# fakerlove1/HPFG

Measured on AMD Instinct MI355X. Metric: labeled+unlabeled images/sec/node, U-Net 224x224 ACDC-shaped (Mean-Teacher step), higher is better.
Workload: dtype bf16x3 (fp32 storage; products as split-bf16 MFMA hi*hi+hi*lo+lo*hi, fp32 accumulate); 1 GPU; mean_teacher_unet_224x224 (BASELINE configs[1]): U-Net 1ch->4cls, 8 labelled + 8 unlabelled per GPU, student fwd+bwd + train-mode teacher fwd + CE/Dice/MSE + SGD + EMA; size=224, hipgraph=True, sync_bn=False, parallelism=dp1, math=bf16x3

## Files before the change

### hpfg_amd/_lib.py

```python
from __future__ import annotations

import ctypes as C
import os
import threading

_HERE = os.path.dirname(os.path.abspath(__file__))
LIB_PATH = os.path.join(_HERE, "lib", "libhpfg_hip.so")

BN_MEAN, BN_RSTD, BN_SCALE, BN_SHIFT, BN_K1, BN_K2, BN_K3, BN_SPARE, BN_ROWS = range(9)
ACT_NONE, ACT_PLAIN, ACT_STRIDED, ACT_BNACT, ACT_BNACT_POOL, ACT_UP2X, ACT_DZ, ACT_SPLIT16, ACT_UPBWD = range(9)
OPT_CONV_THIN, OPT_FIRST_MFMA, OPT_FIRST_WGRAD, OPT_NARROW_DEEP = 0, 1, 2, 3
LOSS_NSUM = 32
ACC_MAX_SHARDS = 8
VERSION = 132
MATH_F32, MATH_BF16X3 = 0, 1


class HipLibraryError(RuntimeError):
    pass


class Act(C.Structure):
    _fields_ = [("z", C.c_void_p), ("bn", C.c_void_p), ("aux", C.c_void_p), ("mode", C.c_int32), ("C", C.c_int32),
                ("Hs", C.c_int32), ("Ws", C.c_int32), ("pstride", C.c_int32), ("aux_pstride", C.c_int32),
                ("bn_stride", C.c_int32), ("bn_coff", C.c_int32), ("sn", C.c_int32), ("sc", C.c_int32), ("sy", C.c_int32),
                ("sx", C.c_int32), ("drop_p", C.c_float), ("drop_seed", C.c_uint32), ("drop_mask", C.c_void_p), ("seed_dev", C.c_void_p),
                ("bn_acc", C.c_void_p), ("bn_gamma", C.c_void_p), ("bn_beta", C.c_void_p), ("bn_count", C.c_float), ("bn_eps", C.c_float),
                ("bn_shards", C.c_int32), ("reserved1", C.c_int32)]


class ConvArgs(C.Structure):
    _fields_ = [("a0", Act), ("a1", Act), ("wpk", C.c_void_p), ("bias", C.c_void_p), ("out", C.c_void_p),
                ("stat_partials", C.c_void_p), ("out_pstride", C.c_int32), ("Cout", C.c_int32), ("CoutPad", C.c_int32),
                ("N", C.c_int32), ("H", C.c_int32), ("W", C.c_int32), ("taps", C.c_int32), ("math", C.c_int32),
                ("bwd_stats", C.c_int32), ("bwd_of", Act), ("out2", C.c_void_p), ("out_split", C.c_int32), ("out2_pstride", C.c_int32),
                ("stat_acc", C.c_void_p), ("stat_shards", C.c_int32), ("reserved2", C.c_int32), ("stage_out", C.c_void_p), ("side_sums", C.c_void_p)]


class WgradArgs(C.Structure):
    _fields_ = [("a0", Act), ("a1", Act), ("g", Act), ("slab", C.c_void_p), ("dw_oihw", C.c_void_p), ("Cin", C.c_int32),
                ("CinPad", C.c_int32), ("Cout", C.c_int32), ("CoutPad", C.c_int32), ("N", C.c_int32), ("H", C.c_int32),
                ("W", C.c_int32), ("taps", C.c_int32), ("S", C.c_int32), ("math", C.c_int32), ("defer_reduce", C.c_int32)]


# ... 165 lines not shown
    "hpfg_neck_pool_fwd": (_i, [_p, _i, _i, _i, _i, _i, _i, _p, _p, _p]),
    "hpfg_neck_pool_bwd": (_i, [_p, _p, _i, _i, _i, _i, _i, _p, _p]),
    "hpfg_l2norm_fwd": (_i, [_p, _i, _i, _i, _i, _i, _p, _p, _p]),
    "hpfg_l2norm_bwd": (_i, [_p, _p, _p, _i, _i, _i, _i, _i, _p, _p, _p]),
    "hpfg_ntxent_rows": (_i, [_p, _i, _f, _p, _p, _p]),
}

_lock = threading.Lock()
_lib = None


def load() -> C.CDLL:
    global _lib
    if _lib is not None:
        return _lib
    with _lock:
        if _lib is not None:
            return _lib
        if not os.path.exists(LIB_PATH):
            raise HipLibraryError(
                f"{LIB_PATH} not found: build it with `python -c 'import __graft_entry__ as g; g.build()'` "
                f"or `make -C hpfg_amd/csrc`. There is no CPU fallback for the HIP path.")
        lib = C.CDLL(LIB_PATH)
        for name, (res, args) in PROTOTYPES.items():
            fn = getattr(lib, name)
            fn.restype = res
            fn.argtypes = args
        if lib.hpfg_version() != VERSION:
            raise HipLibraryError(f"libhpfg_hip.so version {lib.hpfg_version()} != binding version {VERSION}; rebuild")
        if os.environ.get("HPFG_FIRST_WGRAD", "1") == "0":
            lib.hpfg_set_option(OPT_FIRST_WGRAD, 0)
        if os.environ.get("HPFG_NARROW_DEEP") is not None:
            lib.hpfg_set_option(OPT_NARROW_DEEP, int(os.environ["HPFG_NARROW_DEEP"]))
        _lib = lib
    return _lib


def check(rc: int, what: str):
    if rc != 0:
        msg = load().hpfg_last_error().decode("utf-8", "replace")
        raise HipLibraryError(f"{what} failed (rc={rc}): {msg}")


def ptr(t):
    return None if t is None else t.data_ptr()


def none_act() -> Act:
    return Act()
```

### hpfg_amd/csrc/conv_bf16_kernel.h

```cpp
#pragma once
#include <stdlib.h>
#include "stage.h"

namespace hpfg_conv16 {

using namespace hpfg_stage;

template <int TH_, int TW_, int WM_, int WN_, int NI_, int TAPS_, int KC_>
struct Cfg {
  static constexpr int TH = TH_, TW = TW_, WM = WM_, WN = WN_, NI = NI_, TAPS = TAPS_, KC = KC_;
  static constexpr int MI = TH * TW / 16 / WM;
  static constexpr int BN = 16 * NI * WN;
  static constexpr int HALO = TAPS == 9 ? 1 : 0;
  static constexpr int HP = TH + 2 * HALO, WP = TW + 2 * HALO;
  static constexpr int RS = TW == 16 ? WP : (TAPS == 9 ? 24 : 8);
  static constexpr int NSLOT = (HP * RS + 15) / 16 * 16;
  static constexpr int NG = KC / 8;
  static constexpr int PLANE = NSLOT * 16;
  static constexpr int BUF_BYTES = NG * 2 * PLANE;
  static constexpr int KSTEPS = TAPS == 1 ? 1 : (KC == 32 ? 9 : 5);
  static constexpr int NPIECE = HP * WP * NG;
  static constexpr int NLD = (NPIECE + 255) / 256;
  static_assert(WM * WN == 4, "4 waves per workgroup");
  static_assert(256 % NG == 0, "a thread must keep one channel group");
  static_assert(KC == 32 || (KC == 16 && TAPS == 9), "two-tap K packing only for 3x3");
  static_assert(TAPS == 1 || NLD + 2 <= KSTEPS, "stage pipeline must fit into the k-steps of a chunk");
};

__device__ __forceinline__ int clampi(int v, int lo, int hi) { return min(max(v, lo), hi); }

struct Piece {
  int ly, lx, lds, ok;
};
template <class C>
__device__ __forceinline__ Piece make_piece(int tid, int i) {
  Piece q;
  const int idx = tid + i * 256;
  const int pix = idx / C::NG, g = idx % C::NG;
  q.ok = idx < C::NPIECE;
  q.ly = pix / C::WP - C::HALO;
  q.lx = pix % C::WP - C::HALO;
  q.lds = (g * 2) * C::PLANE + ((pix / C::WP) * C::RS + pix % C::WP) * 16;
  return q;
}

template <class C, int KIND = HPFG_KIND_PLAIN, bool SIDE_ON = false>
__device__ __forceinline__ void store_piece(unsigned char* buf, const Piece& q, const f32x4& v0, const f32x4& v1, const HpfgConvArgs* p = nullptr,
                                            bool on = false, int n = 0, int gy = 0, int gx = 0, int c0 = 0, bool ok = false) {
  if (!q.ok) return;
  bf16x8 hi, lo;
  split_piece<KIND>(v0, v1, hi, lo);
  *reinterpret_cast<bf16x8*>(buf + q.lds) = hi;
  *reinterpret_cast<bf16x8*>(buf + q.lds + C::PLANE) = lo;
  if constexpr (SIDE_ON) {
    if (on && ok && q.ly >= 0 && q.ly < C::TH && q.lx >= 0 && q.lx < C::TW) {
      const int ct = p->a0.C + p->a1.C;
      __bf16* d = reinterpret_cast<__bf16*>(p->stage_out) + ((((long)n * p->H + gy) * p->W + gx) * ct + c0) * 2;
      *reinterpret_cast<bf16x8*>(d) = hi;
      *reinterpret_cast<bf16x8*>(d + 8) = lo;
    }
  }
}

template <class C>
__device__ __forceinline__ void load_b(bf16x8 (&bh)[C::NI], bf16x8 (&bl)[C::NI], const bf16x8* wpk, int ks, int ntn, int nt0, int lane) {
#pragma unroll
  for (int j = 0; j < C::NI; ++j) {
    const bf16x8* q = wpk + ((ks * ntn + nt0 + j) * 2) * 64 + lane;
    bh[j] = q[0];
    bl[j] = q[64];
  }
}

template <class C>
__device__ __forceinline__ void conv16_load_bias(const HpfgConvArgs& p, f32x4 (&bias)[C::NI], int lane, int nt0) {
#pragma unroll
  for (int j = 0; j < C::NI; ++j) {
    const int co = (nt0 + j) * 16 + (lane >> 4) * 4;
    bias[j] = f32x4{0.f, 0.f, 0.f, 0.f};
    if (p.bias && co < p.CoutPad) bias[j] = ld4(p.bias, co);
  }
}

template <class C, int BWD_OK = 0>
__device__ __forceinline__ void conv16_store_tile(const HpfgConvArgs& p, f32x4 (&acc)[C::MI][C::NI], f32x4 (&s1)[C::NI], f32x4 (&s2)[C::NI],
                                                  const f32x4 (&bias)[C::NI], int lane, int wm, int nt0, int n, int ty0, int tx0,
                                                  bool reload_bias = false) {
  const int H = p.H, W = p.W;
  const bool vec = (p.Cout & 3) == 0 && (p.out_pstride & 3) == 0 && (p.out2_pstride & 3) == 0;
  const bool bwd = BWD_OK && p.bwd_stats;
  const bool pool = BWD_OK == 2 && bwd;
  ActCtx bcx;
  if (bwd) bcx = make_ctx(p.bwd_of);
#pragma unroll
  for (int j = 0; j < C::NI; ++j) {
    const int co = (nt0 + j) * 16 + (lane >> 4) * 4;
    f32x4 b = bias[j];
    if (reload_bias) {
      b = f32x4{0.f, 0.f, 0.f, 0.f};
      if (p.bias && co < p.CoutPad) b = ld4(p.bias, co);
    }
    f32x4 tsc, tsh;
    if (bwd && co < p.Cout) {
      const float* tb = p.bwd_of.bn + p.bwd_of.bn_coff + co;
      tsc = ld4(tb, HPFG_BN_SCALE * p.bwd_of.bn_stride);
      tsh = ld4(tb, HPFG_BN_SHIFT * p.bwd_of.bn_stride);
// ... 114 lines not shown
      *reinterpret_cast<f32x4*>(ldsf + (1 * C::WM + wm) * C::BN + cl) = s2[j];
    }
  }
  __syncthreads();
  if (tid < 2 * C::BN) {
    const int which = tid / C::BN, cl = tid % C::BN;
    float t = 0.f;
#pragma unroll
    for (int w = 0; w < C::WM; ++w) t += ldsf[(which * C::WM + w) * C::BN + cl];
    const int co = cb * C::BN + cl;
    if (BWD && p.bwd_stats && which == 1 && co < p.Cout) {
      float sg = 0.f;
#pragma unroll
      for (int w = 0; w < C::WM; ++w) sg += ldsf[w * C::BN + cl];
      const float* tb = p.bwd_of.bn + p.bwd_of.bn_coff + co;
      t = tb[HPFG_BN_RSTD * p.bwd_of.bn_stride] * (t - tb[HPFG_BN_MEAN * p.bwd_of.bn_stride] * sg);
    }
    if (p.stat_acc && co < p.Cout)
      hpfg_acc_add(p.stat_acc, p.CoutPad, ((int)blockIdx.z * (int)gridDim.y + (int)blockIdx.y) * (int)gridDim.x + (int)blockIdx.x & (p.stat_shards - 1), which, co, t);
    if (p.stat_partials && co < p.CoutPad) p.stat_partials[((long)row * 2 + which) * p.CoutPad + co] = t;
  }
}

#define HPFG16_MFMA3(ACC, AH, AL, BH, BL)                              \
  ACC = __builtin_amdgcn_mfma_f32_16x16x32_bf16(BH, AH, ACC, 0, 0, 0); \
  ACC = __builtin_amdgcn_mfma_f32_16x16x32_bf16(BL, AH, ACC, 0, 0, 0); \
  ACC = __builtin_amdgcn_mfma_f32_16x16x32_bf16(BH, AL, ACC, 0, 0, 0);

template <class C>
struct UpGeo {
  static constexpr int SH = C::TH / 2 + 3, SW = C::TW / 2 + 3;
  static constexpr int NPIECE = SH * SW * C::NG;
  static constexpr int BYTES = SH * SW * C::KC * 4;
  static_assert(NPIECE <= 256, "one source piece per thread");
};
template <int KIND>
constexpr int eff_nr() { return KIND == HPFG_KIND_CAT ? 2 : RawCount<KIND>::N; }

__device__ __forceinline__ int up_base(int o0, int L) {
  const float r = L > 1 ? (float)(L - 1) / (float)(2 * L - 1) : 0.f;
  return (int)(r * (float)(o0 < 0 ? 0 : o0));
}

template <class C, int KIND>
constexpr int wg_per_cu() {
  return (C::KSTEPS == 5 && C::NI == 1 && RawCount<KIND>::N <= 2) ? 3 : 2;
}

#ifdef HPFG_TRACE
#define HPFG_TR(ID)                                                                                        \
  if (tr_on && tr_i < 255) {                                                                               \
    tr_buf[tr_i++] = ((unsigned long long)(ID) << 56) | (__builtin_amdgcn_s_memtime() & 0xffffffffffffffull); \
  }
#define HPFG_TR_REAL(ID)                                                                                   \
  if (tr_on && tr_i < 255) {                                                                               \
    tr_buf[tr_i++] = ((unsigned long long)(ID) << 56) | (__builtin_amdgcn_s_memrealtime() & 0xffffffffffffffull); \
  }
#else
#define HPFG_TR(ID)
#define HPFG_TR_REAL(ID)
#endif

template <class C, int KIND, int BWD = 0>
__global__ __launch_bounds__(256, (wg_per_cu<C, KIND>())) void conv_bf16x3_kernel(HpfgConvArgs p, int tiles_x, int tiles_y) {
  static_assert(C::TAPS == 9, "persistent kernel is the 3x3 path");
  constexpr int STAT_BYTES = 2 * 4 * C::BN * 4;
  constexpr int NR = eff_nr<KIND>();
  constexpr bool CATK = KIND == HPFG_KIND_CAT;
  constexpr int UP_BYTES = CATK ? UpGeo<C>::BYTES : 0;
  __shared__ __attribute__((aligned(16))) unsigned char lds[2 * C::BUF_BYTES + STAT_BYTES + UP_BYTES];
  float* ldsf = reinterpret_cast<float*>(lds + 2 * C::BUF_BYTES);
  float* ldsU = reinterpret_cast<float*>(lds + 2 * C::BUF_BYTES + STAT_BYTES);
  (void)ldsU;
  constexpr bool TABK = tab_in_lds<KIND>();
  __shared__ __attribute__((aligned(16))) float ldsBN[TABK ? tab_rows<KIND>() * HPFG_BN_CMAX : 4];
  (void)ldsBN;
  const int tid = threadIdx.x, lane = tid & 63, wave = tid >> 6;
  const int wm = wave % C::WM, wn = wave / C::WM;
  const int cb = blockIdx.y;
  const int H = p.H, W = p.W;
  const int ntiles = tiles_x * tiles_y, nwork = ntiles * p.N;
  const ActCtx cx0 = make_ctx(p.a0);
  constexpr bool SIDE = KIND != HPFG_KIND_PLAIN && C::TH == 4;
  const bool dzw = SIDE && p.stage_out != nullptr && cb == 0;
  (void)dzw;
#ifdef HPFG_TRACE
  const bool tr_on = (p.math & 0x2000) && tid == 0;
  unsigned long long* tr_buf = reinterpret_cast<unsigned long long*>(p.stat_partials) + 256 * ((long)blockIdx.y * gridDim.x + blockIdx.x);
  int tr_i = 0;
#endif
  HPFG_TR_REAL(11)
  HPFG_TR(1)

  f32x4 acc[C::MI][C::NI];
#pragma unroll
  for (int m = 0; m < C::MI; ++m)
#pragma unroll
    for (int j = 0; j < C::NI; ++j) acc[m][j] = f32x4{0.f, 0.f, 0.f, 0.f};

  const int kg = lane >> 4;
  const int gl = C::KC == 32 ? kg : (kg & 1);
  int aoff[C::MI];
#pragma unroll
  for (int m = 0; m < C::MI; ++m) {
    const int pxl = (wm * C::MI + m) * 16 + (lane & 15);
    aoff[m] = (gl * 2) * C::PLANE + ((pxl / C::TW) * C::RS + (pxl % C::TW)) * 16;
  }
  int toff[C::KSTEPS];
#pragma unroll
  for (int s = 0; s < C::KSTEPS; ++s) {
    int tap = C::KC == 32 ? s : 2 * s + (kg >> 1);
    tap = tap > 8 ? 8 : tap;
    toff[s] = ((tap / 3) * C::RS + (tap % 3)) * 16;
  }
  Piece pc[C::NLD];
#pragma unroll
  for (int i = 0; i < C::NLD; ++i) pc[i] = make_piece<C>(tid, i);
  const int g8 = (tid % C::NG) * 8;

  const int cin_total = p.a0.C + p.a1.C;
  const int nchunks = (cin_total + C::KC - 1) / C::KC;
  const int ntn = p.CoutPad / 16;
  const int nt0 = (cb * C::WN + wn) * C::NI;
  const bf16x8* wpk = reinterpret_cast<const bf16x8*>(p.wpk);

  const int nx = gridDim.x >= 8 ? 8 : 1;
  const int xg = (int)blockIdx.x % nx, xj = (int)blockIdx.x / nx;
  const int per_x = (nwork + nx - 1) / nx;
  const int wend = (xg + 1) * per_x < nwork ? (xg + 1) * per_x : nwork;
  const int G = ((int)gridDim.x - xg + nx - 1) / nx;
  int w = xg * per_x + xj;
  if (w >= wend) {
    if (p.stat_partials && threadIdx.x < 2 * C::BN) {
      const int co = cb * C::BN + (int)threadIdx.x % C::BN;
      if (co < p.CoutPad) p.stat_partials[((long)blockIdx.x * 2 + (int)threadIdx.x / C::BN) * p.CoutPad + co] = 0.f;
    }
    return;
  }
  int n = w / ntiles, tyi = (w % ntiles) / tiles_x, txi = (w % ntiles) % tiles_x;
  int ty0 = tyi * C::TH, tx0 = txi * C::TW;
  const int gn = G / ntiles, gty = (G % ntiles) / tiles_x, gtx = (G % ntiles) % tiles_x;
  f32x4 s1[C::NI], s2[C::NI];
#pragma unroll
  for (int j = 0; j < C::NI; ++j) {
    s1[j] = f32x4{0.f, 0.f, 0.f, 0.f};
    s2[j] = s1[j];
  }
  constexpr bool TIGHT = C::TAPS == 9 && C::KSTEPS == 5 && C::NI >= 2 && eff_nr<KIND>() >= 4;
  f32x4 bias[C::NI];
  if (!TIGHT) conv16_load_bias<C>(p, bias, lane, nt0);
  Tab tab;
  HPFG_TR(2)
  {
    const int c0 = g8;
    const bool chv = c0 < cin_total;
    const int c0c = chv ? c0 : 0;
    RawPiece<KIND> raw0[C::NLD];
#pragma unroll
    for (int i = 0; i < C::NLD; ++i) {
      const int gy = ty0 + pc[i].ly, gx = tx0 + pc[i].lx;
      const bool ok = pc[i].ok && chv && gy >= 0 && gy < H && gx >= 0 && gx < W;
      issue_piece<KIND>(raw0[i], p.a0, p.a1, cx0, n, clampi(gy, 0, H - 1), clampi(gx, 0, W - 1), c0c, ok);
    }
    if constexpr (TABK) {
      fill_tables_lds<KIND>(p.a0, ldsBN, tid, 256);
      __syncthreads();
      load_tables_lds<KIND>(tab, ldsBN, p.a0, c0c);
    } else {
      load_tables<KIND>(tab, p.a0, c0, chv);
    }
#pragma unroll
    for (int i = 0; i < C::NLD; ++i) {
      const int gy = ty0 + pc[i].ly, gx = tx0 + pc[i].lx;
      const bool ok = pc[i].ok && chv && gy >= 0 && gy < H && gx >= 0 && gx < W;
      f32x4 v0, v1;
      const int gyc = clampi(gy, 0, H - 1), gxc = clampi(gx, 0, W - 1);
      finish_piece<KIND>(v0, v1, raw0[i], tab, p.a0, p.a1, cx0, n, gyc, gxc, c0c, ok);
      store_piece<C, KIND, SIDE>(lds, pc[i], v0, v1, &p, dzw, n, gyc, gxc, c0c, ok);
    }
  }
  constexpr int BR = C::KSTEPS == 5 ? 5 : (C::NI == 1 ? 9 : 3), BD = BR - 1;
  static_assert(C::KSTEPS % BR == 0, "ring size must divide the k-steps of a chunk");
  const int kperiod = nchunks * C::KSTEPS;
  bf16x8 bh[BR][C::NI], bl[BR][C::NI];
#pragma unroll
  for (int d = 0; d < BD; ++d) load_b<C>(bh[d], bl[d], wpk, d % kperiod, ntn, nt0, lane);
  HPFG_TR(3)
  __syncthreads();
  HPFG_TR(4)
  int item = 0;
  while (true) {
    for (int ch = 0; ch < nchunks; ++ch, ++item) {
      const unsigned char* cur = lds + (item & 1) * C::BUF_BYTES;
      unsigned char* nxt = lds + ((item + 1) & 1) * C::BUF_BYTES;
      const bool last_chunk = ch + 1 == nchunks;
      const int w2 = w + G;
      const bool more = !last_chunk || w2 < wend;
      const int nch = last_chunk ? 0 : ch + 1;
      int nn = n, nty = ty0, ntx = tx0;
      if (last_chunk && more) {
        int x2 = txi + gtx, y2 = tyi + gty;
        nn = n + gn;
        if (x2 >= tiles_x) {
          x2 -= tiles_x;
          ++y2;
        }
        if (y2 >= tiles_y) {
          y2 -= tiles_y;
          ++nn;
        }
        nty = y2 * C::TH;
        ntx = x2 * C::TW;
      }
      const int c0n = nch * C::KC + g8;
      const bool chvn = more && c0n < cin_total && !(p.math & 0x400);
      const int c0c = c0n < cin_total ? c0n : 0;
      if constexpr (TABK) load_tables_lds<KIND>(tab, ldsBN, p.a0, c0c);
      else if (!TIGHT || (more && nchunks > 1)) load_tables<KIND>(tab, p.a0, c0c, true);
      constexpr bool DEEP = (NR <= 2 || C::NLD <= 2) && (C::KC != 32 || CATK);
      constexpr int SK = CATK ? HPFG_KIND_BNACT : KIND;
      RawPiece<SK> raw[DEEP ? C::NLD : 2];
      const bool up_next = CATK && nch * C::KC >= p.a0.C;
      f32x4 rawU[2];
      int sy_base = 0, sx_base = 0;
      if (CATK && up_next) {
        using UG = UpGeo<C>;
        sy_base = up_base(nty - 1, p.a1.Hs);
        sx_base = up_base(ntx - 1, p.a1.Ws);
        const int pix = tid / C::NG;
        const int sy = clampi(sy_base + pix / UG::SW, 0, p.a1.Hs - 1), sx = clampi(sx_base + pix % UG::SW, 0, p.a1.Ws - 1);
        const int cu = (c0n < cin_total ? c0n : p.a0.C) - p.a0.C;
        const int off = ((nn * p.a1.Hs + sy) * p.a1.Ws + sx) * p.a1.pstride + cu;
        rawU[0] = ld4(p.a1.z, off);
        rawU[1] = ld4(p.a1.z, off + 4);
      } else if (DEEP) {
#pragma unroll
        for (int i = 0; i < C::NLD; ++i) {
          const int gy = nty + pc[i].ly, gx = ntx + pc[i].lx;
          const bool ok = pc[i].ok && chvn && gy >= 0 && gy < H && gx >= 0 && gx < W;
          issue_piece<SK>(raw[DEEP ? i : 0], p.a0, p.a1, cx0, nn, clampi(gy, 0, H - 1), clampi(gx, 0, W - 1), c0c, ok);
        }
      }
      HPFG_TR(5)
      constexpr int Q = C::KSTEPS * C::MI;
      constexpr int AD0 = wg_per_cu<C, KIND>() == 3 ? 2 : (C::NI == 1 ? 4 : (TIGHT ? 0 : 2));
      constexpr int AD = AD0 < Q ? AD0 : Q;
      constexpr int AR = AD + 1;
      constexpr bool FENCE = !TIGHT;
      bf16x8 ah[AR], al[AR];
#pragma unroll
      for (int q = 0; q < AD; ++q) {
        ah[q % AR] = *reinterpret_cast<const bf16x8*>(cur + aoff[q % C::MI] + toff[q / C::MI]);
        al[q % AR] = *reinterpret_cast<const bf16x8*>(cur + aoff[q % C::MI] + toff[q / C::MI] + C::PLANE);
      }
      if (FENCE) __builtin_amdgcn_sched_barrier(0x216);
#pragma unroll
      for (int q = 0; q < Q; ++q) {
        const int s = q / C::MI, m = q % C::MI;
        if (q + AD < Q) {
          const int q2 = q + AD;
          ah[q2 % AR] = *reinterpret_cast<const bf16x8*>(cur + aoff[q2 % C::MI] + toff[q2 / C::MI]);
          al[q2 % AR] = *reinterpret_cast<const bf16x8*>(cur + aoff[q2 % C::MI] + toff[q2 / C::MI] + C::PLANE);
        }
        if (m == 0) {
          if (!DEEP) {
            if (s >= 2 && s - 2 < C::NLD) {
              const int i = s - 2 < C::NLD ? s - 2 : 0;
              const int gy = nty + pc[i].ly, gx = ntx + pc[i].lx;
              const bool ok = pc[i].ok && chvn && gy >= 0 && gy < H && gx >= 0 && gx < W;
              f32x4 v0, v1;
              finish_piece<SK>(v0, v1, raw[i & 1], tab, p.a0, p.a1, cx0, nn, clampi(gy, 0, H - 1), clampi(gx, 0, W - 1), c0c, ok);
              store_piece<C, SK, SIDE>(nxt, pc[i], v0, v1, &p, dzw, nn, gy, gx, c0c, ok);
            }
            if (s < C::NLD) {
              const int i = s < C::NLD ? s : 0;
              const int gy = nty + pc[i].ly, gx = ntx + pc[i].lx;
              const bool ok = pc[i].ok && chvn && gy >= 0 && gy < H && gx >= 0 && gx < W;
              issue_piece<SK>(raw[i & 1], p.a0, p.a1, cx0, nn, clampi(gy, 0, H - 1), clampi(gx, 0, W - 1), c0c, ok);
            }
          }
          int ksn = ch * C::KSTEPS + s + BD;
          ksn = ksn >= kperiod ? ksn - kperiod : ksn;
          load_b<C>(bh[(s + BD) % BR], bl[(s + BD) % BR], wpk, ksn, ntn, nt0, lane);
        }
#pragma unroll
        for (int j = 0; j < C::NI; ++j) { HPFG16_MFMA3(acc[m][j], ah[q % AR], al[q % AR], bh[s % BR][j], bl[s % BR][j]) }
        if (FENCE) __builtin_amdgcn_sched_barrier(0x216);
      }
      HPFG_TR(6)
      if (CATK && up_next) {
        using UG = UpGeo<C>;
        if (tid < UG::NPIECE) {
          float* d = ldsU + (tid / C::NG) * C::KC + g8;
          *reinterpret_cast<f32x4*>(d) = rawU[0];
          *reinterpret_cast<f32x4*>(d + 4) = rawU[1];
        }
        __syncthreads();
#pragma unroll
        for (int i = 0; i < C::NLD; ++i) {
          const int gy = nty + pc[i].ly, gx = ntx + pc[i].lx;
          const bool ok = pc[i].ok && chvn && gy >= 0 && gy < H && gx >= 0 && gx < W;
          int y0, y1, x0, x1;
          float wy1, wx1;
          up_coord(clampi(gy, 0, H - 1), p.a1.Hs, y0, y1, wy1);
          up_coord(clampi(gx, 0, W - 1), p.a1.Ws, x0, x1, wx1);
          const float wy0 = 1.f - wy1, wx0 = 1.f - wx1;
          const float* r0 = ldsU + ((y0 - sy_base) * UG::SW) * C::KC + g8;
          const float* r1 = ldsU + ((y1 - sy_base) * UG::SW) * C::KC + g8;
          const int o0 = (x0 - sx_base) * C::KC, o1 = (x1 - sx_base) * C::KC;
          const f32x4 a00 = *reinterpret_cast<const f32x4*>(r0 + o0), b00 = *reinterpret_cast<const f32x4*>(r0 + o0 + 4);
          const f32x4 a01 = *reinterpret_cast<const f32x4*>(r0 + o1), b01 = *reinterpret_cast<const f32x4*>(r0 + o1 + 4);
          const f32x4 a10 = *reinterpret_cast<const f32x4*>(r1 + o0), b10 = *reinterpret_cast<const f32x4*>(r1 + o0 + 4);
          const f32x4 a11 = *reinterpret_cast<const f32x4*>(r1 + o1), b11 = *reinterpret_cast<const f32x4*>(r1 + o1 + 4);
          f32x4 v0 = wy0 * (wx0 * a00 + wx1 * a01) + wy1 * (wx0 * a10 + wx1 * a11);
          f32x4 v1 = wy0 * (wx0 * b00 + wx1 * b01) + wy1 * (wx0 * b10 + wx1 * b11);
#pragma unroll
          for (int j = 0; j < 4; ++j) {
            v0[j] = ok ? v0[j] : 0.f;
            v1[j] = ok ? v1[j] : 0.f;
          }
          store_piece<C, HPFG_KIND_PLAIN, SIDE>(nxt, pc[i], v0, v1, &p, dzw, nn, gy, gx, c0c, ok);
        }
      } else if (DEEP) {
#pragma unroll
        for (int i = 0; i < C::NLD; ++i) {
          const int gy = nty + pc[i].ly, gx = ntx + pc[i].lx;
          const bool ok = pc[i].ok && chvn && gy >= 0 && gy < H && gx >= 0 && gx < W;
          f32x4 v0, v1;
          finish_piece<SK>(v0, v1, raw[DEEP ? i : 0], tab, p.a0, p.a1, cx0, nn, clampi(gy, 0, H - 1), clampi(gx, 0, W - 1), c0c, ok);
          store_piece<C, SK, SIDE>(nxt, pc[i], v0, v1, &p, dzw, nn, gy, gx, c0c, ok);
        }
      }
      HPFG_TR(7)
      __syncthreads();
      HPFG_TR(8)
    }
    conv16_store_tile<C, BWD>(p, acc, s1, s2, bias, lane, wm, nt0, n, ty0, tx0, TIGHT);
    HPFG_TR(9)
#pragma unroll
    for (int m = 0; m < C::MI; ++m)
#pragma unroll
      for (int j = 0; j < C::NI; ++j) acc[m][j] = f32x4{0.f, 0.f, 0.f, 0.f};
    w += G;
    if (w >= wend) break;
    txi += gtx;
    tyi += gty;
    n += gn;
    if (txi >= tiles_x) {
      txi -= tiles_x;
      ++tyi;
    }
    if (tyi >= tiles_y) {
      tyi -= tiles_y;
      ++n;
    }
    ty0 = tyi * C::TH;
    tx0 = txi * C::TW;
  }
  conv16_flush_stats<C, BWD>(p, s1, s2, ldsf, tid, lane, wm, wn, cb, (int)blockIdx.x);
  HPFG_TR(10)
  HPFG_TR_REAL(12)
}

template <class C, int KIND, int BWD = 0>
__global__ __launch_bounds__(256) void conv1x1_bf16x3_kernel(HpfgConvArgs p, int tiles_x, int tiles_y) {
  static_assert(C::TAPS == 1, "1x1 path");
  constexpr int STAT_BYTES = 2 * 4 * C::BN * 4;
  constexpr int NR = RawCount<KIND>::N;
  __shared__ __attribute__((aligned(16))) unsigned char lds[C::BUF_BYTES + STAT_BYTES];
  float* ldsf = reinterpret_cast<float*>(lds + C::BUF_BYTES);
  constexpr bool TABK = tab_in_lds<KIND>();
  __shared__ __attribute__((aligned(16))) float ldsBN[TABK ? tab_rows<KIND>() * HPFG_BN_CMAX : 4];
  (void)ldsBN;
  constexpr bool UPB = KIND == HPFG_KIND_UPB;
  __shared__ short upI[UPB ? C::TH + C::TW : 1][HPFG_UPB_TAPS];
  __shared__ float upW[UPB ? C::TH + C::TW : 1][HPFG_UPB_TAPS];
  __shared__ __attribute__((aligned(16))) float upS[UPB ? 256 * 8 : 4];
  (void)upI;
  (void)upW;
  (void)upS;
  const int tid = threadIdx.x, lane = tid & 63, wave = tid >> 6;
  const int wm = wave % C::WM, wn = wave / C::WM;
  const int tile = blockIdx.x, n = blockIdx.y, cb = blockIdx.z;
  const int ty0 = (tile / tiles_x) * C::TH, tx0 = (tile % tiles_x) * C::TW;
  const int H = p.H, W = p.W;
  const ActCtx cx0 = make_ctx(p.a0);
  f32x4 acc[C::MI][C::NI];
#pragma unroll
  for (int m = 0; m < C::MI; ++m)
#pragma unroll
    for (int j = 0; j < C::NI; ++j) acc[m][j] = f32x4{0.f, 0.f, 0.f, 0.f};
  const int kg = lane >> 4;
// ... 111 lines not shown
    if constexpr (UPB) {
      if (side && p.side_sums && tid < C::KC) {
        const int g = tid >> 3, j = tid & 7;
        float tsum = 0.f;
        for (int k = g; k < 256; k += C::NG) tsum += upS[k * 8 + j];
        const int cch = ch * C::KC + tid;
        if (cch < p.a0.C) p.side_sums[(long)wg_row * p.a0.C + cch] = tsum;
      }
    }
#pragma unroll
    for (int m = 0; m < C::MI; ++m) {
      const bf16x8 ah = *reinterpret_cast<const bf16x8*>(lds + aoff[m]);
      const bf16x8 al = *reinterpret_cast<const bf16x8*>(lds + aoff[m] + C::PLANE);
#pragma unroll
      for (int j = 0; j < C::NI; ++j) { HPFG16_MFMA3(acc[m][j], ah, al, bh[j], bl[j]) }
    }
  }
  f32x4 s1[C::NI], s2[C::NI];
#pragma unroll
  for (int j = 0; j < C::NI; ++j) {
    s1[j] = f32x4{0.f, 0.f, 0.f, 0.f};
    s2[j] = s1[j];
  }
  f32x4 bias[C::NI];
  conv16_load_bias<C>(p, bias, lane, nt0);
  conv16_store_tile<C, BWD>(p, acc, s1, s2, bias, lane, wm, nt0, n, ty0, tx0);
  __syncthreads();
  conv16_flush_stats<C, BWD>(p, s1, s2, ldsf, tid, lane, wm, wn, cb, n * (tiles_x * tiles_y) + tile);
}

template <class C, int KIND>
int persistent_grid(const HpfgConvArgs& a) {
  const int tx = (a.W + C::TW - 1) / C::TW, ty = (a.H + C::TH - 1) / C::TH;
  const int lds_bytes = 2 * C::BUF_BYTES + 2 * 4 * C::BN * 4;
  int per_cu = 160 * 1024 / lds_bytes;
  const int reg_cap = wg_per_cu<C, KIND>();
  if (per_cu > reg_cap) per_cu = reg_cap;
  if (per_cu < 1) per_cu = 1;
  const long nwork = (long)tx * ty * a.N;
  const long gy = a.CoutPad / C::BN;
  long cap = 256L * per_cu / (gy > 0 ? gy : 1);
  if (cap < 1) cap = 1;
  const long rounds = (nwork + cap - 1) / cap;
  return (int)((nwork + rounds - 1) / rounds);
}

template <class C, int KIND>
int launch_cfg(const HpfgConvArgs& a, hipStream_t st, int* rows_only) {
  int tx = (a.W + C::TW - 1) / C::TW, ty = (a.H + C::TH - 1) / C::TH;
  if (rows_only) {
    if constexpr (C::TAPS == 9) *rows_only = persistent_grid<C, KIND>(a);
    else *rows_only = tx * ty * a.N;
    return 0;
  }
  if constexpr (C::TAPS == 9) {
    dim3 grid((unsigned)persistent_grid<C, KIND>(a), a.CoutPad / C::BN);
    if (a.stat_acc) HPFG_ACC_CHECK((long)grid.x * grid.y, a.stat_shards, "conv_fwd");
    if constexpr (KIND == HPFG_KIND_DZ || KIND == HPFG_KIND_PLAIN) {
      if constexpr (C::TH == 4) {
        if (a.bwd_stats == 2) {
          hipLaunchKernelGGL((conv_bf16x3_kernel<C, KIND, 2>), grid, dim3(256), 0, st, a, tx, ty);
          return hpfg_launch_status("conv_bf16x3_kernel<bwd stats + pool>");
        }
      }
      if (a.bwd_stats == 2) {
        hpfg_set_error("conv_fwd: bwd_stats == 2 is built for H or W not a multiple of 16");
        return -1;
// ... 5 lines not shown
    }
    hipLaunchKernelGGL((conv_bf16x3_kernel<C, KIND>), grid, dim3(256), 0, st, a, tx, ty);
  } else {
    dim3 grid(tx * ty, a.N, a.CoutPad / C::BN);
    if (a.stat_acc) HPFG_ACC_CHECK((long)grid.x * grid.y * grid.z, a.stat_shards, "conv_fwd(1x1)");
    if constexpr (KIND == HPFG_KIND_DZ || KIND == HPFG_KIND_PLAIN || KIND == HPFG_KIND_UPB) {
      if (a.bwd_stats) {
        hipLaunchKernelGGL((conv1x1_bf16x3_kernel<C, KIND, 1>), grid, dim3(256), 0, st, a, tx, ty);
        return hpfg_launch_status("conv1x1_bf16x3_kernel<bwd stats>");
      }
    }
    hipLaunchKernelGGL((conv1x1_bf16x3_kernel<C, KIND>), grid, dim3(256), 0, st, a, tx, ty);
  }
  return hpfg_launch_status("conv_bf16x3_kernel");
}

template <int KIND, int TAPS>
int conv_dispatch_kind(const HpfgConvArgs& a, hipStream_t st, int* rows_only) {
  const bool big = (a.H % 16 == 0) && (a.W % 16 == 0);
  const int cp = a.CoutPad;
  constexpr int KCB = TAPS == 9 ? 16 : 32;
  if (big) {
    if constexpr (TAPS == 1) {
      if (cp % 64 == 0) return launch_cfg<Cfg<16, 16, 4, 1, 4, TAPS, KCB>, KIND>(a, st, rows_only);
    }
    if (cp % 32 == 0) return launch_cfg<Cfg<16, 16, 4, 1, 2, TAPS, KCB>, KIND>(a, st, rows_only);
    return launch_cfg<Cfg<16, 16, 4, 1, 1, TAPS, KCB>, KIND>(a, st, rows_only);
  }
  if constexpr (TAPS == 9) {
    {
      const long tiles = (long)a.N * ((a.H + 3) / 4) * ((a.W + 15) / 16);
      if (cp % 64 == 0 && tiles * (cp / 64) <= hpfg_opt(HPFG_OPT_NARROW_DEEP))
        return launch_cfg<Cfg<4, 16, 2, 2, 1, TAPS, 32>, KIND>(a, st, rows_only);
    }
    if (cp % 64 == 0) return launch_cfg<Cfg<4, 16, 1, 4, 1, TAPS, 32>, KIND>(a, st, rows_only);
    if (cp % 32 == 0) return launch_cfg<Cfg<4, 16, 2, 2, 1, TAPS, 32>, KIND>(a, st, rows_only);
    return launch_cfg<Cfg<4, 16, 4, 1, 1, TAPS, 32>, KIND>(a, st, rows_only);
  }
  const long nwork = (long)a.N * ((a.H + 7) / 8) * ((a.W + 7) / 8);
  if (cp % 128 == 0 && nwork * (cp / 128) >= 512) return launch_cfg<Cfg<8, 8, 1, 4, 2, TAPS, 32>, KIND>(a, st, rows_only);
  if (cp % 64 == 0 && (nwork * (cp / 64) >= 512 || cp % 32 != 0)) return launch_cfg<Cfg<8, 8, 1, 4, 1, TAPS, 32>, KIND>(a, st, rows_only);
  if (cp % 32 == 0) return launch_cfg<Cfg<8, 8, 2, 2, 1, TAPS, 32>, KIND>(a, st, rows_only);
  return launch_cfg<Cfg<8, 8, 4, 1, 1, TAPS, 32>, KIND>(a, st, rows_only);
}

}

constexpr int HPFG_THIN_NONE = -100;
int hpfg_conv_thin_try(const HpfgConvArgs& a, hipStream_t st, int* rows_only);
int hpfg_conv16_launch_plain(const HpfgConvArgs& a, hipStream_t st, int* rows_only);
int hpfg_conv16_launch_bnact(const HpfgConvArgs& a, hipStream_t st, int* rows_only);
int hpfg_conv16_launch_pool(const HpfgConvArgs& a, hipStream_t st, int* rows_only);
int hpfg_conv16_launch_cat(const HpfgConvArgs& a, hipStream_t st, int* rows_only);
int hpfg_conv16_launch_dz(const HpfgConvArgs& a, hipStream_t st, int* rows_only);
int hpfg_conv16_launch_upb(const HpfgConvArgs& a, hipStream_t st, int* rows_only);
```

### hpfg_amd/csrc/misc.hip

```cpp
#include <stdarg.h>
#include <string.h>
#include "stage.h"

static thread_local char g_err[512] = "";
extern "C" void hpfg_set_error(const char* fmt, ...) {
  va_list ap;
  va_start(ap, fmt);
  vsnprintf(g_err, sizeof(g_err), fmt, ap);
  va_end(ap);
}
extern "C" const char* hpfg_last_error(void) { return g_err; }
extern "C" int hpfg_version(void) { return HPFG_VERSION; }

static int g_opt[HPFG_OPT_COUNT] = {1, 1, 1, 128};
int hpfg_opt(int which) { return which >= 0 && which < HPFG_OPT_COUNT ? g_opt[which] : 0; }
extern "C" int hpfg_set_option(int which, int value) {
  HPFG_ARG_CHECK(which >= 0 && which < HPFG_OPT_COUNT, "set_option: unknown option %d", which);
  const int old = g_opt[which];
  g_opt[which] = value;
  return old;
}

namespace {

__global__ __launch_bounds__(256) void pack_weights_kernel(const HpfgPackDesc* __restrict__ table, long long* __restrict__ counters, int n_counters,
                                                           int* __restrict__ seed_word, int seed_add, long long* __restrict__ zero, long n_zero) {
  if (blockIdx.x == 0 && blockIdx.y == 0) {
    for (int i = threadIdx.x; i < n_counters; i += 256) counters[i] += 1;
    if (threadIdx.x == 0 && seed_word && seed_add) *seed_word = (*seed_word + seed_add) & 0x7FFFFFFF;
  }
  for (long i = ((long)blockIdx.y * gridDim.x + blockIdx.x) * 256 + threadIdx.x; i < n_zero; i += (long)gridDim.x * gridDim.y * 256) zero[i] = 0;
  const HpfgPackDesc d = table[blockIdx.y];
  const long total = (long)d.taps * d.CinPad * d.CoutPad;
  const int nt_f = d.CoutPad / 16, nch_f = d.CinPad / 16;
  const int nt_d = d.CinPad / 16, nch_d = d.CoutPad / 16;
  for (long i = blockIdx.x * 256L + threadIdx.x; i < total; i += (long)gridDim.x * 256) {
    int ks = (int)(i & 3), lane = (int)((i >> 2) & 63);
    long r = i >> 8;
    if (d.wpk_fwd) {
      int nt = (int)(r % nt_f), ch = (int)((r / nt_f) % nch_f), tap = (int)(r / ((long)nt_f * nch_f));
      int co = nt * 16 + (lane & 15), ci = ch * 16 + ks * 4 + (lane >> 4);
      d.wpk_fwd[i] = (co < d.Cout && ci < d.Cin) ? d.w_oihw[((long)co * d.Cin + ci) * d.taps + tap] : 0.f;
    }
    if (d.wpk_dgrad) {
      int nt = (int)(r % nt_d), ch = (int)((r / nt_d) % nch_d), tap = (int)(r / ((long)nt_d * nch_d));
      int co = ch * 16 + ks * 4 + (lane >> 4), ci = nt * 16 + (lane & 15);
      d.wpk_dgrad[i] = (co < d.Cout && ci < d.Cin) ? d.w_oihw[((long)co * d.Cin + ci) * d.taps + (d.taps - 1 - tap)] : 0.f;
// ... 585 lines not shown
```

### include/hpfg_hip.h

```cpp
#ifndef HPFG_HIP_H
#define HPFG_HIP_H

#include <stdint.h>

#ifdef __cplusplus
extern "C" {
#endif

#define HPFG_VERSION 132
enum { HPFG_MATH_F32 = 0, HPFG_MATH_BF16X3 = 1 };

enum { HPFG_BN_MEAN = 0, HPFG_BN_RSTD = 1, HPFG_BN_SCALE = 2, HPFG_BN_SHIFT = 3,
       HPFG_BN_K1 = 4, HPFG_BN_K2 = 5, HPFG_BN_K3 = 6, HPFG_BN_SPARE = 7, HPFG_BN_ROWS = 8 };

enum {
  HPFG_ACT_NONE = 0,
  HPFG_ACT_PLAIN = 1,
  HPFG_ACT_STRIDED = 2,
  HPFG_ACT_BNACT = 3,
  HPFG_ACT_BNACT_POOL = 4,
  HPFG_ACT_UP2X = 5,
  HPFG_ACT_DZ = 6,
  HPFG_ACT_SPLIT16 = 7,
  HPFG_ACT_UPBWD = 8
// ... 57 lines not shown
  int32_t N, H, W, taps;
  int32_t S;
  int32_t math;
  int32_t defer_reduce;
} HpfgWgradArgs;

typedef struct HpfgFusedBwdArgs {
  HpfgConvArgs d;
  HpfgAct xa0, xa1;
  float* slab;
  int32_t Cin, CinPad, Cout, CoutPad;
} HpfgFusedBwdArgs;

typedef struct HpfgSlabDesc {
  const float* slab;
  float* dw_oihw;
  int32_t S, taps, Cin, CinPad, Cout, CoutPad;
} HpfgSlabDesc;

typedef struct HpfgPackDesc {
  const float* w_oihw;
  const float* b;
  float* wpk_fwd;
  float* wpk_dgrad;
  float* bias_pad;
  void* wpk16_fwd;
  void* wpk16_dgrad;
  int32_t Cout, Cin, CoutPad, CinPad, taps;
  int32_t kc;
} HpfgPackDesc;

int hpfg_version(void);
const char* hpfg_last_error(void);
enum { HPFG_OPT_CONV_THIN = 0, HPFG_OPT_FIRST_MFMA = 1, HPFG_OPT_FIRST_WGRAD = 2, HPFG_OPT_NARROW_DEEP = 3, HPFG_OPT_COUNT = 4 };
int hpfg_set_option(int which, int value);

int hpfg_conv3x3_first_fwd(const HpfgAct* x, const float* w_oihw, const float* bias, float* out, float* stat_partials,
                           int N, int H, int W, int Cin, int Cout, void* stream);
int hpfg_conv_first_rows(int N, int H, int W);
int hpfg_conv3x3_first_fwd_acc(const HpfgAct* x, const float* w_oihw, const float* bias, float* out, float* stat_partials, long long* stat_acc,
                               int stat_shards, int N, int H, int W, int Cin, int Cout, void* stream);
int hpfg_conv_fwd(const HpfgConvArgs* args, void* stream);
int hpfg_conv_stat_blocks(int N, int H, int W);
int hpfg_conv_stat_rows(const HpfgConvArgs* args);
int hpfg_bn_fwd_finalize(const float* partials, int nblk, const double* sums, double count, const float* gamma, const float* beta,
                         float* running_mean, float* running_var, float momentum, float eps, float* bn, int C, void* stream);
typedef struct HpfgBnAccDesc {
  const long long* acc;
  const float* gamma;
  const float* beta;
  float* running_mean;
  float* running_var;
  float* bn;
  int32_t C;
  float count;
  int32_t shards;
  int32_t reserved;
} HpfgBnAccDesc;
int hpfg_bn_acc_finalize(const HpfgBnAccDesc* table_dev, const HpfgBnAccDesc* table_host, int nlayers, float momentum, float eps, void* stream);
typedef struct HpfgBnAccBwdDesc {
  long long* acc;
  const float* gamma;
  float* bn;
  float* dgamma;
  float* dbeta;
  int32_t C;
  float count;
// ... 198 lines not shown
```

Baseline: 7591 images/s.

## Split conv K-dimension across wave groups and reduce partial sums through LDS

Adds a K-group variant of the bf16x3 3x3 conv kernel in which two pairs of waves each take alternate 32-channel input chunks, staging 64 channels per pass. Partial accumulators are parked in LDS and summed before the epilogue. The variant is selected for 64-multiple output widths with at least 64 input channels, and by default applies to every tile count. The goal is more input reuse and fewer chunk iterations per workgroup, at the cost of extra LDS, which can lower occupancy, plus a reduction step and a new code path.

Result: slower. 7210 images/s (median of 2 runs) (-5.0%).

```diff
diff --git a/hpfg_amd/_lib.py b/hpfg_amd/_lib.py
--- a/hpfg_amd/_lib.py
+++ b/hpfg_amd/_lib.py
@@ -9,7 +9,7 @@
 
 BN_MEAN, BN_RSTD, BN_SCALE, BN_SHIFT, BN_K1, BN_K2, BN_K3, BN_SPARE, BN_ROWS = range(9)
 ACT_NONE, ACT_PLAIN, ACT_STRIDED, ACT_BNACT, ACT_BNACT_POOL, ACT_UP2X, ACT_DZ, ACT_SPLIT16, ACT_UPBWD = range(9)
-OPT_CONV_THIN, OPT_FIRST_MFMA, OPT_FIRST_WGRAD, OPT_NARROW_DEEP = 0, 1, 2, 3
+OPT_CONV_THIN, OPT_FIRST_MFMA, OPT_FIRST_WGRAD, OPT_NARROW_DEEP, OPT_KGROUPS = 0, 1, 2, 3, 4
 LOSS_NSUM = 32
 ACC_MAX_SHARDS = 8
 VERSION = 132
@@ -241,6 +241,8 @@
             lib.hpfg_set_option(OPT_FIRST_WGRAD, 0)
         if os.environ.get("HPFG_NARROW_DEEP") is not None:
             lib.hpfg_set_option(OPT_NARROW_DEEP, int(os.environ["HPFG_NARROW_DEEP"]))
+        if os.environ.get("HPFG_KGROUPS") is not None:
+            lib.hpfg_set_option(OPT_KGROUPS, int(os.environ["HPFG_KGROUPS"]))
         _lib = lib
     return _lib
 
diff --git a/hpfg_amd/csrc/conv_bf16_kernel.h b/hpfg_amd/csrc/conv_bf16_kernel.h
--- a/hpfg_amd/csrc/conv_bf16_kernel.h
+++ b/hpfg_amd/csrc/conv_bf16_kernel.h
@@ -6,22 +6,25 @@
 
 using namespace hpfg_stage;
 
-template <int TH_, int TW_, int WM_, int WN_, int NI_, int TAPS_, int KC_>
+template <int TH_, int TW_, int WM_, int WN_, int NI_, int TAPS_, int KC_, int NKG_ = 1>
 struct Cfg {
-  static constexpr int TH = TH_, TW = TW_, WM = WM_, WN = WN_, NI = NI_, TAPS = TAPS_, KC = KC_;
+  static constexpr int TH = TH_, TW = TW_, WM = WM_, WN = WN_, NI = NI_, TAPS = TAPS_, KC = KC_, NKG = NKG_;
   static constexpr int MI = TH * TW / 16 / WM;
   static constexpr int BN = 16 * NI * WN;
   static constexpr int HALO = TAPS == 9 ? 1 : 0;
   static constexpr int HP = TH + 2 * HALO, WP = TW + 2 * HALO;
   static constexpr int RS = TW == 16 ? WP : (TAPS == 9 ? 24 : 8);
   static constexpr int NSLOT = (HP * RS + 15) / 16 * 16;
-  static constexpr int NG = KC / 8;
+  static constexpr int KI = KC * NKG;
+  static constexpr int NG = KI / 8;
   static constexpr int PLANE = NSLOT * 16;
   static constexpr int BUF_BYTES = NG * 2 * PLANE;
   static constexpr int KSTEPS = TAPS == 1 ? 1 : (KC == 32 ? 9 : 5);
   static constexpr int NPIECE = HP * WP * NG;
   static constexpr int NLD = (NPIECE + 255) / 256;
-  static_assert(WM * WN == 4, "4 waves per workgroup");
+  static constexpr int PARK_BYTES = NKG == 2 ? TH * TW * BN * 4 : 0;
+  static_assert(WM * WN * NKG == 4, "4 waves per workgroup");
+  static_assert(NKG == 1 || (NKG == 2 && KC == 32 && TAPS == 9 && WM == 1 && MI % 2 == 0), "K-groups: the 3x3 kernel, all pixels per wave");
   static_assert(256 % NG == 0, "a thread must keep one channel group");
   static_assert(KC == 32 || (KC == 16 && TAPS == 9), "two-tap K packing only for 3x3");
   static_assert(TAPS == 1 || NLD + 2 <= KSTEPS, "stage pipeline must fit into the k-steps of a chunk");
@@ -72,6 +75,12 @@
   }
 }
 
+__device__ __forceinline__ void load_b1(bf16x8& bh, bf16x8& bl, const bf16x8* wpk, int ks, int ntn, int nt, int lane) {
+  const bf16x8* q = wpk + ((ks * ntn + nt) * 2) * 64 + lane;
+  bh = q[0];
+  bl = q[64];
+}
+
 template <class C>
 __device__ __forceinline__ void conv16_load_bias(const HpfgConvArgs& p, f32x4 (&bias)[C::NI], int lane, int nt0) {
 #pragma unroll
@@ -252,7 +261,6 @@
   static constexpr int SH = C::TH / 2 + 3, SW = C::TW / 2 + 3;
   static constexpr int NPIECE = SH * SW * C::NG;
   static constexpr int BYTES = SH * SW * C::KC * 4;
-  static_assert(NPIECE <= 256, "one source piece per thread");
 };
 template <int KIND>
 constexpr int eff_nr() { return KIND == HPFG_KIND_CAT ? 2 : RawCount<KIND>::N; }
@@ -288,15 +296,21 @@
   constexpr int NR = eff_nr<KIND>();
   constexpr bool CATK = KIND == HPFG_KIND_CAT;
   constexpr int UP_BYTES = CATK ? UpGeo<C>::BYTES : 0;
-  __shared__ __attribute__((aligned(16))) unsigned char lds[2 * C::BUF_BYTES + STAT_BYTES + UP_BYTES];
+  static_assert(!CATK || UpGeo<C>::NPIECE <= 256, "concat loader: one source piece per thread");
+  constexpr bool KSPLIT = C::NKG == 2;
+  static_assert(!KSPLIT || !CATK, "the concat loader has no K-group form");
+  __shared__ __attribute__((aligned(16))) unsigned char lds[2 * C::BUF_BYTES + STAT_BYTES + UP_BYTES + C::PARK_BYTES];
   float* ldsf = reinterpret_cast<float*>(lds + 2 * C::BUF_BYTES);
   float* ldsU = reinterpret_cast<float*>(lds + 2 * C::BUF_BYTES + STAT_BYTES);
   (void)ldsU;
+  f32x4* ldsP = reinterpret_cast<f32x4*>(lds + 2 * C::BUF_BYTES + STAT_BYTES + UP_BYTES);
+  (void)ldsP;
   constexpr bool TABK = tab_in_lds<KIND>();
   __shared__ __attribute__((aligned(16))) float ldsBN[TABK ? tab_rows<KIND>() * HPFG_BN_CMAX : 4];
   (void)ldsBN;
   const int tid = threadIdx.x, lane = tid & 63, wave = tid >> 6;
-  const int wm = wave % C::WM, wn = wave / C::WM;
+  const int wm = wave % C::WM, wn = KSPLIT ? wave % C::WN : wave / C::WM;
+  const int kgw = KSPLIT ? __builtin_amdgcn_readfirstlane(wave / C::WN) : 0;
   const int cb = blockIdx.y;
   const int H = p.H, W = p.W;
   const int ntiles = tiles_x * tiles_y, nwork = ntiles * p.N;
@@ -319,7 +333,7 @@
     for (int j = 0; j < C::NI; ++j) acc[m][j] = f32x4{0.f, 0.f, 0.f, 0.f};
 
   const int kg = lane >> 4;
-  const int gl = C::KC == 32 ? kg : (kg & 1);
+  const int gl = (C::KC == 32 ? kg : (kg & 1)) + kgw * (C::KC / 8);
   int aoff[C::MI];
 #pragma unroll
   for (int m = 0; m < C::MI; ++m) {
@@ -339,7 +353,9 @@
   const int g8 = (tid % C::NG) * 8;
 
   const int cin_total = p.a0.C + p.a1.C;
-  const int nchunks = (cin_total + C::KC - 1) / C::KC;
+  const int nchunks = (cin_total + C::KI - 1) / C::KI;
+  const int nkc = (cin_total + C::KC - 1) / C::KC;
+  (void)nkc;
   const int ntn = p.CoutPad / 16;
   const int nt0 = (cb * C::WN + wn) * C::NI;
   const bf16x8* wpk = reinterpret_cast<const bf16x8*>(p.wpk);
@@ -399,12 +415,20 @@
       store_piece<C, KIND, SIDE>(lds, pc[i], v0, v1, &p, dzw, n, gyc, gxc, c0c, ok);
     }
   }
-  constexpr int BR = C::KSTEPS == 5 ? 5 : (C::NI == 1 ? 9 : 3), BD = BR - 1;
-  static_assert(C::KSTEPS % BR == 0, "ring size must divide the k-steps of a chunk");
+  constexpr int BR = KSPLIT ? 9 : (C::KSTEPS == 5 ? 5 : (C::NI == 1 ? 9 : 3)), BD = BR - 1;
+  constexpr int BU = KSPLIT ? C::KSTEPS * C::NI : C::KSTEPS;
+  static_assert(BU % BR == 0, "ring size must divide the k-steps of a chunk");
+  static_assert(!KSPLIT || C::NI == 2, "K-group ring: two units per k-step");
   const int kperiod = nchunks * C::KSTEPS;
-  bf16x8 bh[BR][C::NI], bl[BR][C::NI];
-#pragma unroll
-  for (int d = 0; d < BD; ++d) load_b<C>(bh[d], bl[d], wpk, d % kperiod, ntn, nt0, lane);
+  bf16x8 bh[BR][KSPLIT ? 1 : C::NI], bl[BR][KSPLIT ? 1 : C::NI];
+  if constexpr (KSPLIT) {
+    const int kc0 = min(kgw, nkc - 1);
+#pragma unroll
+    for (int u = 0; u < BR - 2; ++u) load_b1(bh[u][0], bl[u][0], wpk, kc0 * C::KSTEPS + u / 2, ntn, nt0 + (u & 1), lane);
+  } else {
+#pragma unroll
+    for (int d = 0; d < BD; ++d) load_b<C>(bh[d], bl[d], wpk, d % kperiod, ntn, nt0, lane);
+  }
   HPFG_TR(3)
   __syncthreads();
   HPFG_TR(4)
@@ -432,7 +456,7 @@
         nty = y2 * C::TH;
         ntx = x2 * C::TW;
       }
-      const int c0n = nch * C::KC + g8;
+      const int c0n = nch * C::KI + g8;
       const bool chvn = more && c0n < cin_total && !(p.math & 0x400);
       const int c0c = c0n < cin_total ? c0n : 0;
       if constexpr (TABK) load_tables_lds<KIND>(tab, ldsBN, p.a0, c0c);
@@ -474,6 +498,45 @@
         al[q % AR] = *reinterpret_cast<const bf16x8*>(cur + aoff[q % C::MI] + toff[q / C::MI] + C::PLANE);
       }
       if (FENCE) __builtin_amdgcn_sched_barrier(0x216);
+      if constexpr (KSPLIT) {
+        static_assert(!DEEP, "K-group form: two-k-step staging ring");
+#pragma unroll
+        for (int s = 0; s < C::KSTEPS; ++s) {
+          if (s >= 2 && s - 2 < C::NLD) {
+            const int i = s - 2 < C::NLD ? s - 2 : 0;
+            const int gy = nty + pc[i].ly, gx = ntx + pc[i].lx;
+            const bool ok = pc[i].ok && chvn && gy >= 0 && gy < H && gx >= 0 && gx < W;
+            f32x4 v0, v1;
+            finish_piece<SK>(v0, v1, raw[i & 1], tab, p.a0, p.a1, cx0, nn, clampi(gy, 0, H - 1), clampi(gx, 0, W - 1), c0c, ok);
+            store_piece<C, SK, SIDE>(nxt, pc[i], v0, v1, &p, dzw, nn, gy, gx, c0c, ok);
+          }
+          if (s < C::NLD) {
+            const int i = s < C::NLD ? s : 0;
+            const int gy = nty + pc[i].ly, gx = ntx + pc[i].lx;
+            const bool ok = pc[i].ok && chvn && gy >= 0 && gy < H && gx >= 0 && gx < W;
+            issue_piece<SK>(raw[i & 1], p.a0, p.a1, cx0, nn, clampi(gy, 0, H - 1), clampi(gx, 0, W - 1), c0c, ok);
+          }
+#pragma unroll
+          for (int d = 0; d < 2; ++d) {
+            const int u = 2 * s + BR - 2 + d, ul = u % BU;
+            const int it = u >= BU ? nch : ch;
+            const int kc = min(it * 2 + kgw, nkc - 1);
+            load_b1(bh[ul % BR][0], bl[ul % BR][0], wpk, kc * C::KSTEPS + ul / 2, ntn, nt0 + (ul & 1), lane);
+          }
+#pragma unroll
+          for (int m = 0; m < C::MI; ++m) {
+            const int q = s * C::MI + m;
+            if (q + AD < Q) {
+              const int q2 = q + AD;
+              ah[q2 % AR] = *reinterpret_cast<const bf16x8*>(cur + aoff[q2 % C::MI] + toff[q2 / C::MI]);
+              al[q2 % AR] = *reinterpret_cast<const bf16x8*>(cur + aoff[q2 % C::MI] + toff[q2 / C::MI] + C::PLANE);
+            }
+#pragma unroll
+            for (int j = 0; j < C::NI; ++j) { HPFG16_MFMA3(acc[m][j], ah[q % AR], al[q % AR], bh[(2 * s + j) % BR][0], bl[(2 * s + j) % BR][0]) }
+            __builtin_amdgcn_sched_barrier(0x216);
+          }
+        }
+      } else {
 #pragma unroll
       for (int q = 0; q < Q; ++q) {
         const int s = q / C::MI, m = q % C::MI;
@@ -506,6 +569,7 @@
 #pragma unroll
         for (int j = 0; j < C::NI; ++j) { HPFG16_MFMA3(acc[m][j], ah[q % AR], al[q % AR], bh[s % BR][j], bl[s % BR][j]) }
         if (FENCE) __builtin_amdgcn_sched_barrier(0x216);
+      }
       }
       HPFG_TR(6)
       if (CATK && up_next) {
@@ -551,11 +615,38 @@
           store_piece<C, SK, SIDE>(nxt, pc[i], v0, v1, &p, dzw, nn, gy, gx, c0c, ok);
         }
       }
+      if constexpr (KSPLIT) {
+        if (last_chunk) {
+          constexpr int MH = C::MI / 2;
+          f32x4* dst = ldsP + (wave * MH * C::NI) * 64 + lane;
+#pragma unroll
+          for (int m = 0; m < MH; ++m)
+#pragma unroll
+            for (int j = 0; j < C::NI; ++j) dst[(m * C::NI + j) * 64] = kgw ? acc[m][j] : acc[MH + m][j];
+        }
+      }
       HPFG_TR(7)
       __syncthreads();
       HPFG_TR(8)
     }
-    conv16_store_tile<C, BWD>(p, acc, s1, s2, bias, lane, wm, nt0, n, ty0, tx0, TIGHT);
+    if constexpr (KSPLIT) {
+      constexpr int MH = C::MI / 2;
+      using CE = Cfg<C::TH, C::TW, 2, 2, C::NI, C::TAPS, C::KC>;
+      static_assert(CE::MI == MH && CE::BN == C::BN, "epilogue view of the K-group form");
+      const f32x4* src = ldsP + (((1 - kgw) * C::WN + wn) * MH * C::NI) * 64 + lane;
+      f32x4 fin[MH][C::NI];
+#pragma unroll
+      for (int m = 0; m < MH; ++m)
+#pragma unroll
+        for (int j = 0; j < C::NI; ++j) {
+          const f32x4 o = src[(m * C::NI + j) * 64];
+          fin[m][j] = kgw ? o + acc[MH + m][j] : acc[m][j] + o;
+        }
+      if (nchunks == 1) __syncthreads();
+      conv16_store_tile<CE, BWD>(p, fin, s1, s2, bias, lane, kgw, nt0, n, ty0, tx0, TIGHT);
+    } else {
+      conv16_store_tile<C, BWD>(p, acc, s1, s2, bias, lane, wm, nt0, n, ty0, tx0, TIGHT);
+    }
     HPFG_TR(9)
 #pragma unroll
     for (int m = 0; m < C::MI; ++m)
@@ -577,7 +668,8 @@
     ty0 = tyi * C::TH;
     tx0 = txi * C::TW;
   }
-  conv16_flush_stats<C, BWD>(p, s1, s2, ldsf, tid, lane, wm, wn, cb, (int)blockIdx.x);
+  if constexpr (KSPLIT) conv16_flush_stats<Cfg<C::TH, C::TW, 2, 2, C::NI, C::TAPS, C::KC>, BWD>(p, s1, s2, ldsf, tid, lane, kgw, wn, cb, (int)blockIdx.x);
+  else conv16_flush_stats<C, BWD>(p, s1, s2, ldsf, tid, lane, wm, wn, cb, (int)blockIdx.x);
   HPFG_TR(10)
   HPFG_TR_REAL(12)
 }
@@ -755,7 +847,7 @@
 template <class C, int KIND>
 int persistent_grid(const HpfgConvArgs& a) {
   const int tx = (a.W + C::TW - 1) / C::TW, ty = (a.H + C::TH - 1) / C::TH;
-  const int lds_bytes = 2 * C::BUF_BYTES + 2 * 4 * C::BN * 4;
+  const int lds_bytes = 2 * C::BUF_BYTES + 2 * 4 * C::BN * 4 + C::PARK_BYTES;
   int per_cu = 160 * 1024 / lds_bytes;
   const int reg_cap = wg_per_cu<C, KIND>();
   if (per_cu > reg_cap) per_cu = reg_cap;
@@ -827,6 +919,10 @@
       const long tiles = (long)a.N * ((a.H + 3) / 4) * ((a.W + 15) / 16);
       if (cp % 64 == 0 && tiles * (cp / 64) <= hpfg_opt(HPFG_OPT_NARROW_DEEP))
         return launch_cfg<Cfg<4, 16, 2, 2, 1, TAPS, 32>, KIND>(a, st, rows_only);
+      if constexpr (KIND == HPFG_KIND_PLAIN || KIND == HPFG_KIND_BNACT || KIND == HPFG_KIND_POOL || KIND == HPFG_KIND_DZ) {
+        if (cp % 64 == 0 && a.a0.C + a.a1.C >= 64 && tiles * (cp / 64) <= hpfg_opt(HPFG_OPT_KGROUPS))
+          return launch_cfg<Cfg<4, 16, 1, 2, 2, TAPS, 32, 2>, KIND>(a, st, rows_only);
+      }
     }
     if (cp % 64 == 0) return launch_cfg<Cfg<4, 16, 1, 4, 1, TAPS, 32>, KIND>(a, st, rows_only);
     if (cp % 32 == 0) return launch_cfg<Cfg<4, 16, 2, 2, 1, TAPS, 32>, KIND>(a, st, rows_only);
diff --git a/hpfg_amd/csrc/misc.hip b/hpfg_amd/csrc/misc.hip
--- a/hpfg_amd/csrc/misc.hip
+++ b/hpfg_amd/csrc/misc.hip
@@ -12,7 +12,7 @@
 extern "C" const char* hpfg_last_error(void) { return g_err; }
 extern "C" int hpfg_version(void) { return HPFG_VERSION; }
 
-static int g_opt[HPFG_OPT_COUNT] = {1, 1, 1, 128};
+static int g_opt[HPFG_OPT_COUNT] = {1, 1, 1, 128, 1 << 20};
 int hpfg_opt(int which) { return which >= 0 && which < HPFG_OPT_COUNT ? g_opt[which] : 0; }
 extern "C" int hpfg_set_option(int which, int value) {
   HPFG_ARG_CHECK(which >= 0 && which < HPFG_OPT_COUNT, "set_option: unknown option %d", which);
diff --git a/include/hpfg_hip.h b/include/hpfg_hip.h
--- a/include/hpfg_hip.h
+++ b/include/hpfg_hip.h
@@ -113,7 +113,7 @@
 
 int hpfg_version(void);
 const char* hpfg_last_error(void);
-enum { HPFG_OPT_CONV_THIN = 0, HPFG_OPT_FIRST_MFMA = 1, HPFG_OPT_FIRST_WGRAD = 2, HPFG_OPT_NARROW_DEEP = 3, HPFG_OPT_COUNT = 4 };
+enum { HPFG_OPT_CONV_THIN = 0, HPFG_OPT_FIRST_MFMA = 1, HPFG_OPT_FIRST_WGRAD = 2, HPFG_OPT_NARROW_DEEP = 3, HPFG_OPT_KGROUPS = 4, HPFG_OPT_COUNT = 5 };
 int hpfg_set_option(int which, int value);
 
 int hpfg_conv3x3_first_fwd(const HpfgAct* x, const float* w_oihw, const float* bias, float* out, float* stat_partials,
```
